# xmed-lab/NEURONS

Hardware: AMD Instinct MI355X
Metric: denoising frames/sec, 16f x 256^2 clip, 50 DDIM steps (higher is better)
Workload: dtype bf16; 1 GPU; BASELINE config 2: 1 clip(s) per call, (1,4,16,32,32) latent, 50 DDIM steps, CFG 8.5 (batch 2), SparseCtrl + temporal U-Net per step, random-init weights; clips_per_gpu=5, ddim_steps=50, hip_graph=True, output_finite=True, attention=bf16

## Files before the change

### neurons_amd/csrc/engine_ops.hip

```cpp
#include "engine.h"
#include <tuple>

using namespace nre;

struct OpScratch { void* ptr = nullptr; size_t cap = 0; };
static bool op_scratch(OpScratch& b, size_t need) {
  if (need <= b.cap) return false;
  if (b.ptr) { HIP_OK(hipDeviceSynchronize()); (void)hipFree(b.ptr); }
  b.ptr = nullptr; b.cap = 0;
  HIP_OK(hipMalloc(&b.ptr, need));
  b.cap = need;
  return true;
}

static std::map<std::tuple<const void*, int, int, int>, bf16*> g_op_fm_cache;
extern "C" void nr_op_fm_cache_clear() {
  (void)hipDeviceSynchronize();
  for (auto& kv : g_op_fm_cache) (void)hipFree(kv.second);
  g_op_fm_cache.clear();
}
static const bf16* op_pack(const NrGemmParams& p, const NrGemmRoute& r, hipStream_t s) {
  if (r.weight_layout == NR_W_ROWMAJOR || r.weight_layout == NR_W_TAP_INNER) return p.w;
  const size_t need = nr_gemm_packed_bytes(r.weight_layout, p.N, p.K);
  if (!need) throw NrError(NR_ERR_STATE, "op_pack: shape has no packed form");
  if (env_is_1("NR_OP_FM_CACHE")) {
    auto it = g_op_fm_cache.find({p.w, r.weight_layout, p.N, p.K});
    if (it == g_op_fm_cache.end()) {
      bf16* d = nullptr;
      HIP_OK(hipMalloc((void**)&d, need));
      LAUNCH_OK(nr_launch_gemm_w_pack(r.weight_layout, p.w, p.N, p.K, d, s));
      it = g_op_fm_cache.emplace(std::make_tuple(p.w, r.weight_layout, p.N, p.K), d).first;
    }
    return it->second;
  }
  static OpScratch scratch[2];
  OpScratch& b = scratch[(r.weight_layout == NR_W_FRAGMAJOR || r.weight_layout == NR_W_FRAGMAJOR_E4M3) ? 0 : 1];
  op_scratch(b, need);
  LAUNCH_OK(nr_launch_gemm_w_pack(r.weight_layout, p.w, p.N, p.K, (bf16*)b.ptr, s));
  return (const bf16*)b.ptr;
}
static void op_gemm(const NrGemmParams& p_arg, hipStream_t s) {
  NrGemmParams p = p_arg;
  p.w8 = env_is_1("NR_W8") ? 1 : 0;
  NrGemmRoute r;
  LAUNCH_OK(nr_gemm_route(&p, &r));
  const bf16* wk = op_pack(p, r, s);
  static OpScratch ws;
  op_scratch(ws, r.ws_bytes);
  LAUNCH_OK(nr_launch_gemm(&p, &r, wk, r.ws_bytes ? (float*)ws.ptr : nullptr, s));
}

extern "C" nr_status nr_op_gemm(nr_stream stream, const void* a, int32_t lda, const void* w, const float* bias,
                                const void* res, int32_t ldr, void* out, int32_t ldo, int32_t M, int32_t N, int32_t K,
                                int32_t geglu) {
  NR_TRY
  NrGemmParams p = nr_gemm_params((const bf16*)a, K, lda, nullptr, 0, 0, M, 1, 1, 1, 1, 0, (const bf16*)w, N, bias, (const bf16*)res, ldr, (bf16*)out, ldo);
  p.geglu = geglu;
  op_gemm(p, (hipStream_t)stream);
  NR_CATCH
}

extern "C" nr_status nr_op_w8_pack(nr_stream stream, const void* w_dev, int32_t N, int32_t K, void* out_dev, int64_t capacity) {
  NR_TRY
  if (!w_dev || !out_dev) throw NrError(NR_ERR_ARG, "null argument");
  const size_t need = nr_gemm_packed_bytes(NR_W_FRAGMAJOR_E4M3, N, K);
  if (!need) throw NrError(NR_ERR_ARG, "e4m3 weights: N must be a multiple of 16 and K of 64");
  if (capacity < (int64_t)need) throw NrError(NR_ERR_ARG, "output buffer too small");
  LAUNCH_OK(nr_launch_gemm_w_pack(NR_W_FRAGMAJOR_E4M3, (const bf16*)w_dev, N, K, (bf16*)out_dev, (hipStream_t)stream));
  NR_CATCH
}

extern "C" nr_status nr_op_gemm2(nr_stream stream, const void* a0, int32_t c0, int32_t lda0, const void* a1, int32_t c1, int32_t lda1,
                                 const void* w, const float* bias, const void* res, int32_t ldr, void* out, int32_t ldo, int32_t M, int32_t N) {
  NR_TRY
  NrGemmParams p = nr_gemm_params((const bf16*)a0, c0, lda0, (const bf16*)a1, c1, lda1, M, 1, 1, 1, 1, 0, (const bf16*)w, N, bias, (const bf16*)res, ldr,
                                  (bf16*)out, ldo);
  op_gemm(p, (hipStream_t)stream);
  NR_CATCH
}

extern "C" nr_status nr_op_ln_gemm(nr_stream stream, const void* a, int32_t lda, const void* w_scaled, const float* ln_c,
                                   const float* bias_folded, float eps, const void* res, int32_t ldr, void* out, int32_t ldo,
                                   int32_t M, int32_t N, int32_t K, int32_t geglu, int32_t act) {
  NR_TRY
  if (!ln_c) throw NrError(NR_ERR_ARG, "ln_c is required");
  NrGemmParams p = nr_gemm_params((const bf16*)a, K, lda, nullptr, 0, 0, M, 1, 1, 1, 1, 0, (const bf16*)w_scaled, N, bias_folded, (const bf16*)res, ldr,
                                  (bf16*)out, ldo);
  p.geglu = geglu; p.ln_c = ln_c; p.ln_eps = eps; p.act = act;
  op_gemm(p, (hipStream_t)stream);
  NR_CATCH
}

extern "C" nr_status nr_op_gemm_ex(nr_stream stream, const void* a, int32_t lda, const void* w, const float* bias, const float* ln_c,
                                   float ln_eps, const float* rowvec, int32_t rowvec_div, int32_t rowvec_mod, int32_t rowvec_ld,
                                   const void* res, int32_t ldr, void* out, int32_t ldo, int32_t M, int32_t N, int32_t K, int32_t geglu,
                                   int32_t act, float out_scale) {
  NR_TRY
  NrGemmParams p = nr_gemm_params((const bf16*)a, K, lda, nullptr, 0, 0, M, 1, 1, 1, 1, 0, (const bf16*)w, N, bias, (const bf16*)res, ldr, (bf16*)out, ldo);
  p.out_scale = out_scale; p.geglu = geglu; p.act = act;
  p.rowvec = rowvec; p.rowvec_div = rowvec_div > 0 ? rowvec_div : 1; p.rowvec_mod = rowvec_mod; p.rowvec_ld = rowvec_ld;
  p.ln_c = ln_c; p.ln_eps = ln_eps;
  op_gemm(p, (hipStream_t)stream);
  NR_CATCH
}

extern "C" nr_status nr_op_conv3x3(nr_stream stream, const void* x0, int32_t c0, const void* x1, int32_t c1, int32_t nimg,
                                   int32_t H, int32_t W, int32_t stride, int32_t ups, const void* w, const float* bias,
                                   const float* rowvec, int32_t rowvec_div, const void* res, void* out, int32_t Cout) {
  NR_TRY
  NrGemmParams p = nr_gemm_params((const bf16*)x0, c0, c0, (const bf16*)x1, c1, c1, nimg, H, W, 3, stride, ups, (const bf16*)w, Cout, bias, (const bf16*)res,
                                  Cout, (bf16*)out, Cout);
  p.rowvec = rowvec; p.rowvec_div = rowvec_div > 0 ? rowvec_div : 1; p.rowvec_ld = Cout;
  op_gemm(p, (hipStream_t)stream);
  NR_CATCH
}

extern "C" nr_status nr_op_conv3x3_ups_phase(nr_stream stream, const void* x, int32_t Cin, int32_t nimg, int32_t H, int32_t W, const void* wp,
                                             const float* bias, void* out, int32_t Cout) {
  NR_TRY
  if (!x || !wp || !out) throw NrError(NR_ERR_ARG, "null argument");
  NrGemmParams p = nr_gemm_params((const bf16*)x, Cin, Cin, nullptr, 0, 0, nimg, H, W, 3, 1, 2, (const bf16*)wp, Cout, bias, nullptr, 0, (bf16*)out, Cout);
  op_gemm(p, (hipStream_t)stream);
  NR_CATCH
}
extern "C" nr_status nr_ups_phase_weights(const float* w_tap, int32_t Cout, int32_t Cin, void* out) {
  NR_TRY
  if (!w_tap || !out || Cout < 1 || Cin < 1) throw NrError(NR_ERR_ARG, "bad argument");
  nr_ups_phase_pack(w_tap, (size_t)9 * Cin, 1, (size_t)Cin, Cout, Cin, (uint16_t*)out);
  NR_CATCH
}

extern "C" nr_status nr_op_condembed_in(nr_stream stream, const float* cond, const float* mask, int32_t c0, int32_t nsrc, int32_t F, int32_t H,
                                        int32_t W, const int32_t* fmap, int32_t nframes, const float* w, const float* bias, int32_t Cout,
                                        void* out) {
  NR_TRY
  if (!fmap) throw NrError(NR_ERR_ARG, "fmap is null");
  LAUNCH_OK(nr_launch_condembed_in(cond, mask, c0, nsrc, F, H, W, fmap, nframes, w, bias, Cout, (bf16*)out, (hipStream_t)stream));
  NR_CATCH
}

extern "C" nr_status nr_op_condembed_conv(nr_stream stream, const void* x, int32_t nimg, int32_t H, int32_t W, int32_t Cin, int32_t stride,
                                          const void* wfm, const float* bias, int32_t Cout, int32_t silu, void* out) {
  NR_TRY
  LAUNCH_OK(nr_launch_condembed_conv((const bf16*)x, nimg, H, W, Cin, stride, (const bf16*)wfm, bias, Cout, silu, (bf16*)out,
                                     (hipStream_t)stream));
  NR_CATCH
}

extern "C" nr_status nr_op_conv3x3_tap_inner(nr_stream stream, const void* x0, int32_t c0, int32_t nimg, int32_t H, int32_t W, const void* w,
                                             const float* bias, const float* rowvec, int32_t rowvec_div, const void* res, void* out,
                                             int32_t Cout) {
  NR_TRY
  NrGemmParams p = nr_gemm_params((const bf16*)x0, c0, c0, nullptr, 0, 0, nimg, H, W, 3, 1, 0, (const bf16*)w, Cout, bias, (const bf16*)res, Cout, (bf16*)out,
                                  Cout);
  p.tap_inner = 1;
  p.rowvec = rowvec; p.rowvec_div = rowvec_div > 0 ? rowvec_div : 1; p.rowvec_ld = Cout;
  op_gemm(p, (hipStream_t)stream);
  NR_CATCH
}

extern "C" nr_status nr_op_groupnorm(nr_stream stream, const void* x0, int32_t c0, const void* x1, int32_t c1, int32_t nimg,
                                     int32_t hw, int32_t groups, const float* gamma, const float* beta, float eps,
                                     int32_t silu, float* partial_ws, void* out) {
  NR_TRY
  NrGnParams p = nr_gn_params((const bf16*)x0, c0, c0, (const bf16*)x1, c1, c1, nimg, hw, groups, gamma, beta, eps, silu, partial_ws, (bf16*)out,
                              c0 + (x1 ? c1 : 0));
  NrGnRoute r;
  if (const int rc = nr_gn_route(&p, &r)) throw NrError(NR_ERR_UNSUPPORTED, "nr_gn_route -> " + std::to_string(rc) + ": no kernel serves this shape, nr_launch_groupnorm not called");
  LAUNCH_OK(nr_launch_groupnorm(&p, &r, (hipStream_t)stream));
  NR_CATCH
}

extern "C" nr_status nr_op_layernorm(nr_stream stream, const void* x, void* out, int32_t M, int32_t C, const float* gamma,
                                     const float* beta, float eps, const float* pe, int32_t pe_hw, int32_t pe_F) {
  NR_TRY
  LAUNCH_OK(nr_launch_layernorm((const bf16*)x, C, (bf16*)out, C, M, C, gamma, beta, eps, pe, pe_hw > 0 ? pe_hw : 1,
                                pe_F > 0 ? pe_F : 1, (hipStream_t)stream));
  NR_CATCH
}

extern "C" nr_status nr_op_attention(nr_stream stream, int32_t mode, const void* qp, const void* kvp, void* outp,
                                     int32_t nimg, int32_t L, int32_t Lk, int32_t C, int32_t heads, int32_t frames,
                                     int32_t kv_div) {
  NR_TRY
  const int fp8_flag = (mode & 8) ? 1 : 0;
  const int causal_flag = (mode & 16) ? 1 : 0;
  mode &= 7;
  if (causal_flag && (mode != 0 || fp8_flag)) throw NrError(NR_ERR_ARG, "causal attention: mode 0 only");
  if (mode > 2) throw NrError(NR_ERR_ARG, "bad attention mode");
  const NrAttnParams p = nr_attn_params(mode, (const bf16*)qp, (const bf16*)kvp, (bf16*)outp, mode == 1 ? C : 3 * C, 2 * C, C, nimg, L, Lk, C, heads, frames, kv_div,
                                        causal_flag, fp8_flag);
  NrAttnRoute r;
  if (const int rc = nr_attn_route(&p, &r)) throw NrError(NR_ERR_UNSUPPORTED, "nr_attn_route -> " + std::to_string(rc) + ": no kernel serves this shape, nr_launch_attention not called");
  LAUNCH_OK(nr_launch_attention(&p, &r, (hipStream_t)stream));
  NR_CATCH
}
// ... 103 lines not shown
```

### neurons_amd/csrc/gemm_route.h

```cpp
#pragma once
#include "common.h"
#include <cstdlib>
#include <initializer_list>

inline bool env_not_0(const char* name) {
  const char* v = getenv(name);
  return !(v && v[0] == '0');
}

inline int nr_plan_rows(const NrGemmParams& p) { return (p.plan_m > 0 && p.plan_m < p.M) ? p.plan_m : p.M; }

inline int nr_lds_opt_in(unsigned long long& mask, std::initializer_list<const void*> fns, size_t bytes) {
  int dev = 0;
  (void)hipGetDevice(&dev);
  const unsigned long long bit = 1ull << (dev & 63);
  if (mask & bit) return 0;
  for (const void* fn : fns)
    if (hipFuncSetAttribute(fn, hipFuncAttributeMaxDynamicSharedMemorySize, (int)bytes) != hipSuccess) return 2;
  mask |= bit;
  return 0;
}

enum NrGemmClass { NR_GEMM_SMALLM, NR_GEMM_LIN160, NR_GEMM_ROWPANEL, NR_GEMM_G8P, NR_GEMM_TILED, NR_GEMM_NCLASS };
inline const char* const nr_gemm_class_name[NR_GEMM_NCLASS] = {"smallm", "lin160", "rowpanel", "gemm8p", "tiled"};
enum NrWeightLayout { NR_W_ROWMAJOR, NR_W_TAP_INNER, NR_W_FRAGMAJOR, NR_W_LIN160, NR_W_LIN128Q, NR_W_FRAGMAJOR_E4M3 };

struct TiledPlan { int bm, bn, splitk, stages, waves, adma, lin; };
struct SmallmPlan { int nt, G, J, C; };
struct Lin160Plan { int form, big, J, cgmajor; };
struct RowPanelPlan { int nsplit; };
struct G8pPlan { int nt, phases; };

struct NrGemmRoute {
  int cls;
  int weight_layout;
  int m_fast;
  size_t ws_bytes;
  TiledPlan tiled;
  SmallmPlan smallm;
  Lin160Plan lin160;
  RowPanelPlan rowpanel;
  G8pPlan g8p;
};
```

### neurons_amd/csrc/lin160.hip

```cpp
#include "launchers.h"
#include "device_prims.h"
#include <cstdlib>

namespace {

NR_STAMP_BUF(lin160_stamp_buf, 512, 128);
#define L1_STAMP(slot) NR_STAMP_PUT(lin160_stamp_buf, slot)
#ifdef NR_STAMP_FINE
#define Q_STAMPW(slot) NR_STAMP_PUT_AT((threadIdx.x & 63) == 0 && (wave == 0 || wave == 4) && blockIdx.x < 256, lin160_stamp_buf, blockIdx.x + (wave ? 256 : 0), slot)
#else
#define Q_STAMPW(slot) do { } while (0)
#endif

constexpr int L1_BN = 160, L1_NT = 10;
constexpr int L1_W_STAGE = 24 * 1024;
constexpr int L1_NS = 3;

struct NrLin160Params {
  const bf16* x; int lda;
  const bf16* stream;
  const float* bias;
  const bf16* res; int ldr;
  bf16* out; int ldo;
  int M, N, K;
  const float* ln_c; float ln_eps;
  int norot;
};

template <int BM, int MODE = 0>
__global__ __launch_bounds__(512) void lin160_kernel(NrLin160Params p) {
  constexpr bool GLN = MODE == 1;
  static_assert(!GLN || BM == 128, "the GEGLU variant pairs the (value, gate) tiles inside one wave");
  constexpr int RT = BM / 16;
  constexpr int NTW = BM == 128 ? L1_NT : L1_NT / 2;
  constexpr int A_STAGE = BM * 128;
  constexpr int A_PW = BM == 128 ? 2 : 1;
  constexpr int STAGE = L1_W_STAGE + A_STAGE;
  constexpr int PPW = 3 + A_PW;
  extern __shared__ __attribute__((aligned(16))) unsigned char smem[];

  const int tid = threadIdx.x;
  const int lane = tid & 63;
  const int wave = __builtin_amdgcn_readfirstlane(tid >> 6);
  const int fr = lane & 15, fg = lane >> 4;
  const int rt = BM == 128 ? wave : (wave & 3);
  const int n0 = BM == 128 ? 0 : (wave >> 2) * NTW;

  L1_STAMP(0);
  const int NCB = p.N / L1_BN, S = p.K >> 6;
  const int nrg = p.M / BM;
  int rg, cb;
  if ((nrg & 7) == 0) { const int j = blockIdx.x >> 3; cb = j % NCB; rg = (j / NCB) * 8 + (int)(blockIdx.x & 7); }
  else { cb = (int)(blockIdx.x % NCB); rg = blockIdx.x / NCB; }
  const int r0 = rg * BM;
  const int rot = p.norot ? 0 : rg % S;

  const unsigned lds0 = nr_lds_addr(smem);
  const char* wsrc = reinterpret_cast<const char*>(p.stream) + (size_t)cb * ((size_t)S * L1_W_STAGE) + (size_t)(wave * 3) * 1024 + (size_t)lane * 16;
  const bf16* arow;
  {
    const int r = lane >> 2;
    arow = p.x + (size_t)(r0 + 16 * rt + r) * p.lda + (((lane & 3) ^ ((-(r >> 2)) & 3)) << 3);
  }
  auto issue_piece = [&](int s, int slot, int i) {
    const unsigned dst = lds0 + (unsigned)(slot * STAGE);
    int st = s + rot; if (st >= S) st -= S;
    if (i < 3) nr_glds16(wsrc + (size_t)st * L1_W_STAGE + (size_t)i * 1024, dst + (unsigned)((wave * 3 + i) * 1024));
    else {
      const int kk = BM == 128 ? i - 3 : (wave >> 2);
      nr_glds16(arow + 64 * st + 32 * kk, dst + (unsigned)(L1_W_STAGE + (kk * RT + rt) * 1024));
    }
  };
#pragma unroll
  for (int s = 0; s < L1_NS - 1; ++s)
#pragma unroll
    for (int i = 0; i < PPW; ++i) issue_piece(s, s, i);

  L1_STAMP(1);
  f32x4 acc[NTW];
#pragma unroll
  for (int n = 0; n < NTW; ++n) acc[n] = f32x4{0.f, 0.f, 0.f, 0.f};
  float s1 = 0.f, s2 = 0.f;
  const bf16x2 one2 = {(bf16)1.0f, (bf16)1.0f};
  const unsigned wl = (unsigned)(n0 * 1024 + lane * 16);
  const unsigned al = (unsigned)(L1_W_STAGE + rt * 1024 + fr * 64 + ((fg ^ ((-(fr >> 2)) & 3)) << 4));

  int slot = 0;
  for (int s = 0; s < S; ++s) {
    if (s + 1 < S) nr_wait_vmcnt<(L1_NS - 2) * PPW>(); else nr_wait_vmcnt<0>();
    if (s < 40) L1_STAMP(2 + 3 * s);
    __builtin_amdgcn_s_barrier();
    if (s < 40) L1_STAMP(3 + 3 * s);
    const int s_next = s + L1_NS - 1;
    const bool pf = s_next < S;
    int pslot = slot + L1_NS - 1; if (pslot >= L1_NS) pslot -= L1_NS;
    const unsigned char* base = smem + slot * STAGE;
#pragma unroll
    for (int kk = 0; kk < 2; ++kk) {
      const bf16x8 xa = *(const bf16x8*)(base + al + kk * (RT * 1024));
      if constexpr (GLN) {
#pragma unroll
        for (int e = 0; e < 4; ++e) {
          const bf16x2 pr = {xa[2 * e], xa[2 * e + 1]};
          s1 = __builtin_amdgcn_fdot2_f32_bf16(pr, one2, s1, false);
          s2 = __builtin_amdgcn_fdot2_f32_bf16(pr, pr, s2, false);
        }
      }
      bf16x8 w[NTW];
#pragma unroll
      for (int n = 0; n < NTW; ++n) w[n] = *(const bf16x8*)(base + (unsigned)((kk * L1_NT + n) * 1024) + wl);
      if (pf) {
        if (kk == 0) { issue_piece(s_next, pslot, 0); issue_piece(s_next, pslot, 1); }
        else { issue_piece(s_next, pslot, 2); issue_piece(s_next, pslot, 3); if (A_PW == 2) issue_piece(s_next, pslot, 4); }
      }
      __builtin_amdgcn_sched_barrier(0);
#pragma unroll
      for (int n = 0; n < NTW; ++n) acc[n] = __builtin_amdgcn_mfma_f32_16x16x32_bf16(w[n], xa, acc[n], 0, 0, 0);
      __builtin_amdgcn_sched_barrier(0);
    }
    if (s < 40) L1_STAMP(4 + 3 * s);
    slot = slot + 1 == L1_NS ? 0 : slot + 1;
  }
  L1_STAMP(125);

  if constexpr (GLN) {
    const float inv_k = 1.0f / (float)p.K;
    const float mu = nr_rows_sum(s1) * inv_k;
    const float rstd = rsqrtf(fmaxf(nr_rows_sum(s2) * inv_k - mu * mu, 0.f) + p.ln_eps);
    const int row = r0 + 16 * rt + fr;
    const int nb = cb * L1_BN + 4 * fg;
    bf16* orow = p.out + (size_t)row * p.ldo + cb * (L1_BN / 2) + 4 * fg;
#pragma unroll
    for (int i = 0; i < L1_NT / 2; ++i) {
      const int nv = nb + 32 * i, ng = nv + 16;
      const f32x4 cv = *(const f32x4*)(p.ln_c + nv), cg = *(const f32x4*)(p.ln_c + ng);
      const f32x4 bv = *(const f32x4*)(p.bias + nv), bg = *(const f32x4*)(p.bias + ng);
      bf16x4 o;
#pragma unroll
      for (int e = 0; e < 4; ++e) {
        const float v = (acc[2 * i][e] - mu * cv[e]) * rstd + bv[e];
        const float g = (acc[2 * i + 1][e] - mu * cg[e]) * rstd + bg[e];
        o[e] = (bf16)(v * gelu_erf_fast(g));
      }
      nr_store8(orow + 16 * i, o);
    }
    L1_STAMP(126);
    return;
  }
  const int row = r0 + 16 * rt + fr;
  const int cbase = cb * L1_BN + 16 * n0;
  bf16* orow = p.out + (size_t)row * p.ldo + cbase;
  const bf16* rrow = p.res ? p.res + (size_t)row * p.ldr + cbase : nullptr;
#pragma unroll
  for (int k = 0; k < NTW / 2; ++k) {
    f32x4 lo = acc[2 * k], hi = acc[2 * k + 1];
// ... 133 lines not shown
      f32x4 a1 = {0.f, 0.f, 0.f, 0.f}, a2 = {0.f, 0.f, 0.f, 0.f};
#pragma unroll
      for (int ks = 0; ks < KSL; ++ks) {
        a1 = __builtin_amdgcn_mfma_f32_16x16x32_bf16(ones, xb[rt][ks], a1, 0, 0, 0);
        a2 = __builtin_amdgcn_mfma_f32_16x16x32_bf16(xb[rt][ks], xb[rt][ks], a2, 0, 0, 0);
      }
      const int e_d = fr & 3;
      float d = e_d == 0 ? a2[0] : e_d == 1 ? a2[1] : e_d == 2 ? a2[2] : a2[3];
      d = (fg == (fr >> 2)) ? d : 0.f;
      sx[rt] = a1[0];
      sq2[rt] = nr_rows_sum(d);
    }
    if constexpr (KSPLIT) {
      float* xs = reinterpret_cast<float*>(smem + NS * Q_STAGE);
      if (fg == 0) {
#pragma unroll
        for (int rt = 0; rt < 2; ++rt) { xs[((wave * 2 + rt) * 2 + 0) * 16 + fr] = sx[rt]; xs[((wave * 2 + rt) * 2 + 1) * 16 + fr] = sq2[rt]; }
      }
      __builtin_amdgcn_s_barrier();
#pragma unroll
      for (int rt = 0; rt < 2; ++rt) { sx[rt] += xs[(((wave ^ 4) * 2 + rt) * 2 + 0) * 16 + fr]; sq2[rt] += xs[(((wave ^ 4) * 2 + rt) * 2 + 1) * 16 + fr]; }
    }
#pragma unroll
    for (int rt = 0; rt < 2; ++rt) {
      mu[rt] = sx[rt] * (1.0f / K);
      rstd[rt] = rsqrtf(fmaxf(sq2[rt] * (1.0f / K) - mu[rt] * mu[rt], 0.f) + p.ln_eps);
    }
  }
  L1_STAMP(127);
  nr_wait_vmcnt<0>();
  __builtin_amdgcn_s_barrier();
  L1_STAMP(1);

  const unsigned wl = (unsigned)((KSPLIT ? 16 * ch : 4 * ch) * 1024 + lane * 16);
  const unsigned oofs = (unsigned)row0 * (unsigned)p.ldo + (unsigned)((KSPLIT ? (GEGLU ? 16 * ch : 32 * ch) : (GEGLU ? 32 * ch : 64 * ch)) + 4 * fg);
  bf16x8 w[4];
#pragma unroll
  for (int n = 0; n < 4; ++n) w[n] = *(const bf16x8*)(smem + (unsigned)(n * 1024) + wl);
  f32x4 acc[2][4];
  auto epilogue = [&](int jb) {
    const int cb = cg * J + jb;
    constexpr int NF = KSPLIT ? 2 : 4;
    const float* tc = tab + jb * BN + 16 * (NF * ch) + 4 * fg;
    const float* tb = tc + J * BN;
    if constexpr (KSPLIT) {
      f32x4* ex = reinterpret_cast<f32x4*>(smem + NS * Q_STAGE);
#pragma unroll
      for (int rt = 0; rt < 2; ++rt)
#pragma unroll
        for (int nn = 0; nn < 2; ++nn) {
          f32x4 theirs;
#pragma unroll
          for (int e = 0; e < 4; ++e) theirs[e] = ch ? acc[rt][nn][e] : acc[rt][2 + nn][e];
          ex[((wave * 2 + rt) * 2 + nn) * 64 + lane] = theirs;
        }
      __builtin_amdgcn_s_barrier();
      const f32x4 c0 = *(const f32x4*)(tc), c1 = *(const f32x4*)(tc + 16), b0 = *(const f32x4*)(tb), b1 = *(const f32x4*)(tb + 16);
#pragma unroll
      for (int rt = 0; rt < 2; ++rt) {
        const f32x4 o0 = ex[(((wave ^ 4) * 2 + rt) * 2 + 0) * 64 + lane], o1 = ex[(((wave ^ 4) * 2 + rt) * 2 + 1) * 64 + lane];
        bf16x4 r0, r1;
#pragma unroll
        for (int e = 0; e < 4; ++e) {
          const float t0 = ((ch ? acc[rt][2][e] : acc[rt][0][e]) + o0[e] - mu[rt] * c0[e]) * rstd[rt] + b0[e];
          const float t1 = ((ch ? acc[rt][3][e] : acc[rt][1][e]) + o1[e] - mu[rt] * c1[e]) * rstd[rt] + b1[e];
          if constexpr (GEGLU) r0[e] = (bf16)(t0 * gelu_erf_fast(t1));
          else { r0[e] = (bf16)t0; r1[e] = (bf16)t1; }
        }
        bf16* orow = p.out + (oofs + (unsigned)(16 * rt) * (unsigned)p.ldo + (unsigned)(cb * (GEGLU ? BN / 2 : BN)));
        nr_store8(orow, r0);
        if constexpr (!GEGLU) nr_store8(orow + 16, r1);
      }
    } else if constexpr (GEGLU) {
#pragma unroll
      for (int i = 0; i < NF / 2; ++i) {
        const f32x4 cv = *(const f32x4*)(tc + 32 * i), cgv = *(const f32x4*)(tc + 32 * i + 16);
        const f32x4 bv = *(const f32x4*)(tb + 32 * i), bg = *(const f32x4*)(tb + 32 * i + 16);
#pragma unroll
        for (int rt = 0; rt < 2; ++rt) {
          bf16x4 o;
#pragma unroll
          for (int e = 0; e < 4; ++e) {
            const float v = (acc[rt][2 * i][e] - mu[rt] * cv[e]) * rstd[rt] + bv[e];
            const float gt = (acc[rt][2 * i + 1][e] - mu[rt] * cgv[e]) * rstd[rt] + bg[e];
            o[e] = (bf16)(v * gelu_erf_fast(gt));
          }
          nr_store8(p.out + (oofs + (unsigned)(16 * rt) * (unsigned)p.ldo + (unsigned)(cb * (BN / 2) + 16 * i)), o);
        }
      }
    } else {
#pragma unroll
      for (int n = 0; n < NF; ++n) {
        const f32x4 c4 = *(const f32x4*)(tc + 16 * n), b4 = *(const f32x4*)(tb + 16 * n);
#pragma unroll
        for (int rt = 0; rt < 2; ++rt) {
          bf16x4 o;
#pragma unroll
          for (int e = 0; e < 4; ++e) o[e] = (bf16)((acc[rt][n][e] - mu[rt] * c4[e]) * rstd[rt] + b4[e]);
          nr_store8(p.out + (oofs + (unsigned)(16 * rt) * (unsigned)p.ldo + (unsigned)(cb * BN + 16 * n)), o);
        }
      }
    }
  };
  const f32x4 zero4 = {0.f, 0.f, 0.f, 0.f};
  int g = 0, slot = 0;
  for (int j = 0; j < J; ++j) {
#pragma unroll
    for (int st = 0; st < S; ++st) {
      const int nslot = slot + 1 == NS ? 0 : slot + 1;
#pragma unroll
      for (int kk = 0; kk < 4; ++kk) {
        const unsigned char* nbase;
        if (kk < 3) nbase = smem + slot * Q_STAGE + (kk + 1) * (NTB * 1024);
        else {
          nr_wait_vmcnt<(NS - 2) * 4>();
          asm volatile("s_waitcnt lgkmcnt(0)" ::: "memory");
          if (g < 40) L1_STAMP(2 + 3 * g);
          __builtin_amdgcn_s_barrier();
          if (g < 40) L1_STAMP(3 + 3 * g);
          nbase = smem + nslot * Q_STAGE;
        }
        __builtin_amdgcn_sched_barrier(0);
        if (kk == 0) {
#pragma unroll
          for (int i = 0; i < 4; ++i) issue_piece(g + NS - 1, i);
        }
        __builtin_amdgcn_sched_barrier(0);
#pragma unroll
        for (int n = 0; n < 4; ++n) {
#pragma unroll
          for (int rt = 0; rt < 2; ++rt)
            acc[rt][n] = __builtin_amdgcn_mfma_f32_16x16x32_bf16(w[n], xb[rt][4 * st + kk], (st == 0 && kk == 0) ? zero4 : acc[rt][n], 0, 0, 0);
          __builtin_amdgcn_sched_barrier(0);
          w[n] = *(const bf16x8*)(nbase + (unsigned)(n * 1024) + wl);
          __builtin_amdgcn_sched_barrier(0);
        }
      }
      if (g < 40) L1_STAMP(4 + 3 * g);
      ++g;
      slot = nslot;
    }
    epilogue(j);
    if constexpr (KSPLIT) {
      __builtin_amdgcn_sched_barrier(0);
#pragma unroll
      for (int n = 0; n < 4; ++n) w[n] = *(const bf16x8*)(smem + slot * Q_STAGE + (unsigned)(n * 1024) + wl);
    }
  }
  L1_STAMP(125);
  nr_wait_vmcnt<0>();
  L1_STAMP(126);
}

__global__ __launch_bounds__(256) void lin128q_w_pack_kernel(const bf16* __restrict__ w, bf16* __restrict__ stream, int N, int K, int BN, int KPS) {
  const int S = K / (32 * KPS), CH_STAGE = Q_STAGE / 16, NTB = BN / 16;
  const long long idx = (long long)blockIdx.x * 256 + threadIdx.x;
  if (idx >= (long long)(N / BN) * S * CH_STAGE) return;
  const int cb = (int)(idx / ((long long)S * CH_STAGE));
  int c = (int)(idx - (long long)cb * S * CH_STAGE);
  const int st = c / CH_STAGE;
  c -= st * CH_STAGE;
  const int kk = c / (NTB * 64), n = (c / 64) % NTB, lane = c & 63;
  *(bf16x8*)(stream + (size_t)idx * 8) = *(const bf16x8*)(w + (size_t)(cb * BN + 16 * n + (lane & 15)) * K + 32 * (KPS * st + kk) + 8 * (lane >> 4));
}

}

#ifdef NR_STAMP
extern "C" int nr_lin160_stamp_read(void* dst, size_t bytes, int clear) { return nr_stamp_read_buf(lin160_stamp_buf, dst, bytes, clear); }
#endif

extern "C" size_t nr_lin160_stream_bytes(int N, int K) { return (N % L1_BN == 0 && K % 64 == 0) ? (size_t)(N / L1_BN) * (K / 64) * L1_W_STAGE : 0; }

extern "C" int nr_lin160_panel_rule(int Mp, int N, int K) {
  static const bool off = !env_not_0("NR_LIN160") || !env_not_0("NR_LIN160_PANEL");
  static const bool off1280 = !env_not_0("NR_LIN160_PANEL_K1280");
  static const int maxm = getenv("NR_LIN160_PANEL_MAXM") ? atoi(getenv("NR_LIN160_PANEL_MAXM")) : (1 << 30);
  if (off || Mp < 2048 || Mp > maxm || N < 3 * K) return 0;
  if (K == 640) return Mp >= 4096 && N % Q_BN == 0;
  if (K == 1280) return !off1280 && N % 64 == 0;
  return 0;
}
extern "C" size_t nr_lin128q_stream_bytes(int N, int K) {
  if (K == 640) return N % Q_BN == 0 ? (size_t)N * K * sizeof(bf16) : 0;
  if (K == 1280) return N % 64 == 0 ? (size_t)N * K * sizeof(bf16) : 0;
  return 0;
}
extern "C" int nr_launch_lin128q_w_pack(const bf16* w, int N, int K, bf16* stream, hipStream_t s) {
  const long long total = (long long)(nr_lin128q_stream_bytes(N, K) / 16);
  if (!total) return 1;
  hipLaunchKernelGGL(lin128q_w_pack_kernel, dim3((unsigned)((total + 255) / 256)), dim3(256), 0, s, w, stream, N, K, K == 1280 ? 64 : Q_BN, K == 1280 ? 8 : 4);
  return 0;
}

extern "C" bool lin160_plan(const NrGemmParams& p, Lin160Plan* pl) {
  static const bool off = !env_not_0("NR_LIN160");
  const int Mp = nr_plan_rows(p);
  *pl = Lin160Plan{0, 0, 0, 0};
  const bool ln_wide = p.ln_c && p.bias && p.ksize == 1 && p.stride == 1 && !p.ups && !p.a1 && !p.c1 && !p.rowvec && !p.act && !p.out_f32 && !p.res &&
                       p.out_scale == 1.0f && p.K == p.c0 && p.M % 128 == 0 && p.lda0 % 8 == 0 && p.ldo % 4 == 0;
  if (ln_wide && nr_lin160_panel_rule(Mp, p.N, p.K) &&
      (long long)p.M * p.ldo < (1ll << 31)) {
    const bool ksplit = p.K == 1280;
    const int bn = ksplit ? 64 : Q_BN, ncq = p.N / bn, S = 5, nrg = p.M / 128, ns = ksplit ? 3 : Q_NS;
    static const int j_force = getenv("NR_LIN160_PANEL_J") ? atoi(getenv("NR_LIN160_PANEL_J")) : 0;
    int J = 0; long long best = 0;
    for (int c = 1; c <= 16 && c <= ncq; ++c) {
      if (ncq % c != 0 || c * S < ns - 1) continue;
      const long long wgs = (long long)nrg * (ncq / c), cost = ((wgs + 255) / 256) * (c * S + 6);
      if (!J || cost <= best) { J = c; best = cost; }
    }
    if (j_force > 0 && ncq % j_force == 0 && j_force <= 16) J = j_force;
    pl->form = 4; pl->J = J;
    if (J) {
      static const int cg_force = getenv("NR_LIN160_PANEL_CGMAJOR") ? atoi(getenv("NR_LIN160_PANEL_CGMAJOR")) : -1;
      const int NCG = ncq / J;
      const double wb = 2.0 * p.N * (double)p.K, xb = 2.0 * p.M * (double)p.K;
      const bool can = NCG % 8 == 0 || 8 % NCG == 0;
      const double by_rg = 8.0 * wb + xb;
      const double by_cg = (NCG % 8 == 0 ? 1.0 : 8.0 / NCG) * wb + (NCG % 8 == 0 ? 8.0 : (double)NCG) * xb;
      pl->cgmajor = (can && by_cg < by_rg) ? 1 : 0;
      if (cg_force >= 0) pl->cgmajor = cg_force && can;
    }
    return true;
  }
  static const bool gln_on = env_not_0("NR_LIN160_GEGLU");
  if (!off && gln_on && ln_wide && p.geglu && p.K == 1280 && p.N % L1_BN == 0 && p.N >= 8192 && Mp <= 1024 && (long long)(Mp / 128) * (p.N / L1_BN) >= 192) {
    pl->form = 2;
    return true;
  }
  if (off || p.ksize != 1 || p.stride != 1 || p.ups || p.a1 || p.c1 || p.geglu || p.ln_c || p.rowvec || p.act || p.out_f32 || p.tap_inner) return false;
  if (p.out_scale != 1.0f || p.K != p.c0 || (p.K != 640 && p.K != 1280) || p.N % L1_BN != 0 || p.N > 1280) return false;
  if (p.M % 64 != 0 || Mp < 2048) return false;
  if (p.lda0 % 8 != 0 || p.ldo % 8 != 0 || (p.res && p.ldr % 8 != 0)) return false;
  if (Mp > 8192) return false;
  pl->form = 1;
  pl->big = p.M % 128 == 0 && (long long)(Mp / 128) * (p.N / L1_BN) >= 256;
  return true;
}

extern "C" int nr_launch_lin160_w_pack(const bf16* w, int N, int K, bf16* stream, hipStream_t s) {
  const long long total = (long long)(nr_lin160_stream_bytes(N, K) / 16);
  if (!total) return 1;
  hipLaunchKernelGGL(lin160_w_pack_kernel, dim3((unsigned)((total + 255) / 256)), dim3(256), 0, s, w, stream, N, K);
  return 0;
}

extern "C" int nr_launch_lin160(const NrGemmParams* pp, const Lin160Plan* pl, const bf16* stream, hipStream_t s) {
  const NrGemmParams& g = *pp;
  if (!stream) return 1;
  if (pl->form == 4) {
    const bool ksplit = g.K == 1280;
    if (!g.ln_c || !g.bias || (g.K != 640 && !ksplit) || g.M % 128 != 0 || (long long)g.M * g.ldo >= (1ll << 31)) return 1;
    const int bn = ksplit ? 64 : Q_BN, ncq = g.N / bn, nrg = g.M / 128, ns = ksplit ? 3 : Q_NS, J = pl->J;
    if (g.N % bn != 0 || J < 1 || J > 16 || ncq % J != 0) return 1;
    NrLin128QParams q;
    q.x = g.a0; q.lda = g.lda0; q.stream = stream; q.ln_c = g.ln_c; q.bias = g.bias; q.ln_eps = g.ln_eps; q.out = g.out; q.ldo = g.ldo; q.M = g.M; q.N = g.N; q.norot = g.plan_m > 0 ? 1 : 0;
    q.J = J; q.NCG = ncq / J; q.cgmajor = pl->cgmajor;
    const size_t shm_max = (size_t)Q_NS * Q_STAGE + 2 * 16 * Q_BN * sizeof(float);
    const size_t shm = (size_t)ns * Q_STAGE + (ksplit ? 32 * 1024 : 0) + (size_t)2 * J * bn * sizeof(float);
    typedef void (*kern_t)(NrLin128QParams);
    static const kern_t ks[4] = {lin128q_kernel<20, true>, lin128q_kernel<20, false>, lin128q_kernel<40, true, true>, lin128q_kernel<40, false, true>};
    static unsigned long long done[4] = {};
    const int ki = (ksplit ? 2 : 0) + (g.geglu ? 0 : 1);
    if (const int rc = nr_lds_opt_in(done[ki], {(const void*)ks[ki]}, shm_max)) return rc;
    hipLaunchKernelGGL(ks[ki], dim3((unsigned)(nrg * q.NCG)), dim3(512), shm, s, q);
    return 0;
  }
  if (g.M % 64 != 0 || g.N % L1_BN != 0 || g.K % 64 != 0 || g.K / 64 < L1_NS) return 1;
  NrLin160Params p;
  p.x = g.a0; p.lda = g.lda0; p.stream = stream; p.bias = g.bias; p.res = g.res; p.ldr = g.ldr; p.out = g.out; p.ldo = g.ldo; p.M = g.M; p.N = g.N; p.K = g.K; p.norot = g.plan_m > 0 ? 1 : 0;
  const int ncb = g.N / L1_BN;
  p.ln_c = g.ln_c; p.ln_eps = g.ln_eps;
  const bool gln = pl->form == 2, big = gln || pl->big;
  if (gln != (g.geglu != 0) || (gln && (!g.ln_c || !g.bias)) || (big && g.M % 128 != 0)) return 1;
  typedef void (*kern_t)(NrLin160Params);
  static const kern_t ks[3] = {lin160_kernel<128, 1>, lin160_kernel<128, 0>, lin160_kernel<64, 0>};
  const int ki = gln ? 0 : (big ? 1 : 2), rows = big ? 128 : 64;
  const size_t shm = (size_t)L1_NS * (L1_W_STAGE + rows * 128);
  static unsigned long long done[3] = {};
  if (const int rc = nr_lds_opt_in(done[ki], {(const void*)ks[ki]}, shm)) return rc;
  hipLaunchKernelGGL(ks[ki], dim3((unsigned)((g.M / rows) * ncb)), dim3(512), shm, s, p);
  return 0;
}
```

Measured before the change: 20.97 frames/s.

## Add LN-fused panel GEMM variant that overlaps row statistics with first weight block

Adds a new lin128q kernel variant for the non-GEGLU LayerNorm-fused panel GEMM. It loads the whole activation panel once and computes the row mean and variance with MFMA reductions (a ones vector and x·x) inside the first column block's main loop. Load issue and vmcnt waits are staged with compile-time counts so the statistics prologue overlaps with weight streaming instead of running serially. It is on by default for non-GEGLU shapes, and also adds env knobs for a minimum M and deterministic batch planning. The cost is more register pressure, extra LDS for the K-split statistics exchange, and fragile hand-tuned waitcnt arithmetic.

```diff
diff --git a/neurons_amd/csrc/engine_ops.hip b/neurons_amd/csrc/engine_ops.hip
--- a/neurons_amd/csrc/engine_ops.hip
+++ b/neurons_amd/csrc/engine_ops.hip
@@ -42,6 +42,7 @@
 static void op_gemm(const NrGemmParams& p_arg, hipStream_t s) {
   NrGemmParams p = p_arg;
   p.w8 = env_is_1("NR_W8") ? 1 : 0;
+  if (env_is_1("NR_DETERMINISTIC_BATCH")) p.plan_m = p.M;
   NrGemmRoute r;
   LAUNCH_OK(nr_gemm_route(&p, &r));
   const bf16* wk = op_pack(p, r, s);
diff --git a/neurons_amd/csrc/gemm_route.h b/neurons_amd/csrc/gemm_route.h
--- a/neurons_amd/csrc/gemm_route.h
+++ b/neurons_amd/csrc/gemm_route.h
@@ -27,7 +27,7 @@
 
 struct TiledPlan { int bm, bn, splitk, stages, waves, adma, lin; };
 struct SmallmPlan { int nt, G, J, C; };
-struct Lin160Plan { int form, big, J, cgmajor; };
+struct Lin160Plan { int form; union { int big; int early; }; int J, cgmajor; };
 struct RowPanelPlan { int nsplit; };
 struct G8pPlan { int nt, phases; };
 
diff --git a/neurons_amd/csrc/lin160.hip b/neurons_amd/csrc/lin160.hip
--- a/neurons_amd/csrc/lin160.hip
+++ b/neurons_amd/csrc/lin160.hip
@@ -1,6 +1,7 @@
 #include "launchers.h"
 #include "device_prims.h"
 #include <cstdlib>
+#include <type_traits>
 
 namespace {
 
@@ -440,6 +441,272 @@
   L1_STAMP(126);
 }
 
+
+template <int... I, class F> __device__ __forceinline__ void q_static_for(std::integer_sequence<int, I...>, F&& f) { (f(std::integral_constant<int, I>{}), ...); }
+constexpr int q_grp(int s, int S) { return s < S ? 12 : 4; }
+constexpr int q_younger(int from, int to, int S) { int n = 0; for (int s = from; s <= to; ++s) n += q_grp(s, S); return n; }
+constexpr int q_hi(int st, int S, int NS) { return st < S - 1 ? st + 2 : S + NS - 2; }
+constexpr int q_wait_x(int st, int kk, int S, int NS) { return 6 - 2 * kk + q_younger(st + 1, q_hi(st, S, NS), S); }
+constexpr int q_wait_w(int st, int S, int NS) { return (st + 1 < S ? 8 : 0) + q_younger(st + 2, q_hi(st, S, NS), S); }
+
+template <int KS, bool GEGLU, bool KSPLIT = false>
+__global__ __launch_bounds__(512) void lin128q_early_kernel(NrLin128QParams p) {
+  constexpr int K = 32 * KS;
+  constexpr int KSL = KSPLIT ? KS / 2 : KS;
+  constexpr int KPS = KSPLIT ? 8 : 4;
+  constexpr int S = KS / KPS;
+  constexpr int BN = KSPLIT ? 64 : Q_BN, NTB = BN / 16;
+  constexpr int NS = KSPLIT ? 3 : Q_NS;
+  constexpr int XCH = KSPLIT ? 32 * 1024 : 0;
+  static_assert(KSL == 20 && S == 5, "20 k-steps per wave in 5 stages of 4");
+  extern __shared__ __attribute__((aligned(16))) unsigned char smem[];
+  const int tid = threadIdx.x;
+  const int lane = tid & 63;
+  const int wave = __builtin_amdgcn_readfirstlane(tid >> 6);
+  const int fr = lane & 15, fg = lane >> 4;
+  const int rp = wave & 3, ch = wave >> 2;
+  L1_STAMP(0);
+  const int J = p.J;
+  int rg, cg;
+  const int nrg = p.M >> 7;
+  if (!p.cgmajor && (nrg & 7) == 0) { const int i = blockIdx.x >> 3; cg = i % p.NCG; rg = (i / p.NCG) * 8 + (int)(blockIdx.x & 7); }
+  else { cg = (int)(blockIdx.x % p.NCG); rg = (int)(blockIdx.x / p.NCG); }
+  const int row0 = rg * 128 + 32 * rp + fr;
+  const int rot = p.norot ? 0 : rg % S;
+  const int G = J * S;
+
+  const unsigned lds0 = nr_lds_addr(smem);
+  const char* wbase = reinterpret_cast<const char*>(p.stream) + (size_t)cg * J * ((size_t)S * Q_STAGE) + (size_t)(wave * 4) * 1024 + (size_t)lane * 16;
+  auto issue_piece = [&](int g, int i) {
+    const int gs = g < G ? g : G - 1;
+    const int j = gs / S;
+    int st = gs - j * S + rot; if (st >= S) st -= S;
+    nr_glds16(wbase + ((size_t)j * S + st) * Q_STAGE + (size_t)i * 1024, lds0 + (unsigned)((g % NS) * Q_STAGE + (wave * 4 + i) * 1024));
+  };
+  float* tab = reinterpret_cast<float*>(smem + NS * Q_STAGE + XCH);
+  bf16x8 xb[2][KSL];
+  const bf16* xr[2];
+#pragma unroll
+  for (int rt = 0; rt < 2; ++rt) xr[rt] = p.x + (size_t)(row0 + 16 * rt) * p.lda + 8 * fg + (KSPLIT ? 128 * ch : 0);
+  auto issue_panel = [&](int st) {
+    int sq = st + rot; if (sq >= S) sq -= S;
+#pragma unroll
+    for (int kk = 0; kk < 4; ++kk)
+#pragma unroll
+      for (int rt = 0; rt < 2; ++rt)
+        asm volatile("global_load_dwordx4 %0, %1, off" : "=v"(xb[rt][4 * st + kk]) : "v"(xr[rt] + 32 * (KPS * sq + kk)) : "memory");
+  };
+  float mu[2], rstd[2], sx[2], sq2[2];
+  f32x4 sa1[2] = {{0.f, 0.f, 0.f, 0.f}, {0.f, 0.f, 0.f, 0.f}}, sa2[2] = {{0.f, 0.f, 0.f, 0.f}, {0.f, 0.f, 0.f, 0.f}};
+  bf16x8 ones;
+#pragma unroll
+  for (int e = 0; e < 8; ++e) ones[e] = (bf16)1.0f;
+  auto stats_step = [&](int rt, int ks) {
+    sa1[rt] = __builtin_amdgcn_mfma_f32_16x16x32_bf16(ones, xb[rt][ks], sa1[rt], 0, 0, 0);
+    sa2[rt] = __builtin_amdgcn_mfma_f32_16x16x32_bf16(xb[rt][ks], xb[rt][ks], sa2[rt], 0, 0, 0);
+  };
+  auto stats_rows = [&]() {
+#pragma unroll
+    for (int rt = 0; rt < 2; ++rt) {
+      const int e_d = fr & 3;
+      float d = e_d == 0 ? sa2[rt][0] : e_d == 1 ? sa2[rt][1] : e_d == 2 ? sa2[rt][2] : sa2[rt][3];
+      d = (fg == (fr >> 2)) ? d : 0.f;
+      sx[rt] = sa1[rt][0];
+      sq2[rt] = nr_rows_sum(d);
+    }
+  };
+  float* xs = reinterpret_cast<float*>(smem + NS * Q_STAGE + XCH + 2 * J * BN * sizeof(float));
+  auto stats_put = [&]() {
+    if (fg == 0) {
+#pragma unroll
+      for (int rt = 0; rt < 2; ++rt) { xs[((wave * 2 + rt) * 2 + 0) * 16 + fr] = sx[rt]; xs[((wave * 2 + rt) * 2 + 1) * 16 + fr] = sq2[rt]; }
+    }
+  };
+  auto stats_get = [&]() {
+#pragma unroll
+    for (int rt = 0; rt < 2; ++rt) { sx[rt] += xs[(((wave ^ 4) * 2 + rt) * 2 + 0) * 16 + fr]; sq2[rt] += xs[(((wave ^ 4) * 2 + rt) * 2 + 1) * 16 + fr]; }
+  };
+  auto stats_final = [&]() {
+#pragma unroll
+    for (int rt = 0; rt < 2; ++rt) {
+      mu[rt] = sx[rt] * (1.0f / K);
+      rstd[rt] = rsqrtf(fmaxf(sq2[rt] * (1.0f / K) - mu[rt] * mu[rt], 0.f) + p.ln_eps);
+    }
+  };
+
+  {
+    const int n4 = (J * BN) >> 2, tq = tid < n4 ? tid : n4 - 1;
+    f32x4 tc, tb;
+    asm volatile("global_load_dwordx4 %0, %1, off" : "=v"(tc) : "v"(p.ln_c + cg * J * BN + 4 * tq) : "memory");
+    asm volatile("global_load_dwordx4 %0, %1, off" : "=v"(tb) : "v"(p.bias + cg * J * BN + 4 * tq) : "memory");
+#pragma unroll
+    for (int g = 0; g <= q_hi(-1, S, NS); ++g) {
+#pragma unroll
+      for (int i = 0; i < 4; ++i) issue_piece(g, i);
+      issue_panel(g);
+    }
+    L1_STAMP(122);
+    asm volatile("s_waitcnt vmcnt(%2)" : "+v"(tc), "+v"(tb) : "n"(q_wait_w(-1, S, NS)) : "memory");
+    if (tid < n4) { *(f32x4*)(tab + 4 * tid) = tc; *(f32x4*)(tab + J * BN + 4 * tid) = tb; }
+    L1_STAMP(123);
+    __builtin_amdgcn_s_barrier();
+  }
+  L1_STAMP(1);
+
+  const unsigned wl = (unsigned)((KSPLIT ? 16 * ch : 4 * ch) * 1024 + lane * 16);
+  const unsigned oofs = (unsigned)row0 * (unsigned)p.ldo + (unsigned)((KSPLIT ? (GEGLU ? 16 * ch : 32 * ch) : (GEGLU ? 32 * ch : 64 * ch)) + 4 * fg);
+  bf16x8 w[4];
+#pragma unroll
+  for (int n = 0; n < 4; ++n) w[n] = *(const bf16x8*)(smem + (unsigned)(n * 1024) + wl);
+  f32x4 acc[2][4];
+  auto epilogue = [&](int jb, auto with_stats) {
+    constexpr bool STATS = decltype(with_stats)::value;
+    if constexpr (STATS) stats_rows();
+    if constexpr (STATS && !KSPLIT) { stats_final(); L1_STAMP(127); }
+    const int cb = cg * J + jb;
+    constexpr int NF = KSPLIT ? 2 : 4;
+    const float* tc = tab + jb * BN + 16 * (NF * ch) + 4 * fg;
+    const float* tb = tc + J * BN;
+    if constexpr (KSPLIT) {
+      f32x4* ex = reinterpret_cast<f32x4*>(smem + NS * Q_STAGE);
+#pragma unroll
+      for (int rt = 0; rt < 2; ++rt)
+#pragma unroll
+        for (int nn = 0; nn < 2; ++nn) {
+          f32x4 theirs;
+#pragma unroll
+          for (int e = 0; e < 4; ++e) theirs[e] = ch ? acc[rt][nn][e] : acc[rt][2 + nn][e];
+          ex[((wave * 2 + rt) * 2 + nn) * 64 + lane] = theirs;
+        }
+      if constexpr (STATS) stats_put();
+      __builtin_amdgcn_s_barrier();
+      if constexpr (STATS) { stats_get(); stats_final(); L1_STAMP(127); }
+      const f32x4 c0 = *(const f32x4*)(tc), c1 = *(const f32x4*)(tc + 16), b0 = *(const f32x4*)(tb), b1 = *(const f32x4*)(tb + 16);
+#pragma unroll
+      for (int rt = 0; rt < 2; ++rt) {
+        const f32x4 o0 = ex[(((wave ^ 4) * 2 + rt) * 2 + 0) * 64 + lane], o1 = ex[(((wave ^ 4) * 2 + rt) * 2 + 1) * 64 + lane];
+        bf16x4 r0, r1;
+#pragma unroll
+        for (int e = 0; e < 4; ++e) {
+          const float t0 = ((ch ? acc[rt][2][e] : acc[rt][0][e]) + o0[e] - mu[rt] * c0[e]) * rstd[rt] + b0[e];
+          const float t1 = ((ch ? acc[rt][3][e] : acc[rt][1][e]) + o1[e] - mu[rt] * c1[e]) * rstd[rt] + b1[e];
+          if constexpr (GEGLU) r0[e] = (bf16)(t0 * gelu_erf_fast(t1));
+          else { r0[e] = (bf16)t0; r1[e] = (bf16)t1; }
+        }
+        bf16* orow = p.out + (oofs + (unsigned)(16 * rt) * (unsigned)p.ldo + (unsigned)(cb * (GEGLU ? BN / 2 : BN)));
+        nr_store8(orow, r0);
+        if constexpr (!GEGLU) nr_store8(orow + 16, r1);
+      }
+    } else if constexpr (GEGLU) {
+#pragma unroll
+      for (int i = 0; i < NF / 2; ++i) {
+        const f32x4 cv = *(const f32x4*)(tc + 32 * i), cgv = *(const f32x4*)(tc + 32 * i + 16);
+        const f32x4 bv = *(const f32x4*)(tb + 32 * i), bg = *(const f32x4*)(tb + 32 * i + 16);
+#pragma unroll
+        for (int rt = 0; rt < 2; ++rt) {
+          bf16x4 o;
+#pragma unroll
+          for (int e = 0; e < 4; ++e) {
+            const float v = (acc[rt][2 * i][e] - mu[rt] * cv[e]) * rstd[rt] + bv[e];
+            const float gt = (acc[rt][2 * i + 1][e] - mu[rt] * cgv[e]) * rstd[rt] + bg[e];
+            o[e] = (bf16)(v * gelu_erf_fast(gt));
+          }
+          nr_store8(p.out + (oofs + (unsigned)(16 * rt) * (unsigned)p.ldo + (unsigned)(cb * (BN / 2) + 16 * i)), o);
+        }
+      }
+    } else {
+#pragma unroll
+      for (int n = 0; n < NF; ++n) {
+        const f32x4 c4 = *(const f32x4*)(tc + 16 * n), b4 = *(const f32x4*)(tb + 16 * n);
+#pragma unroll
+        for (int rt = 0; rt < 2; ++rt) {
+          bf16x4 o;
+#pragma unroll
+          for (int e = 0; e < 4; ++e) o[e] = (bf16)((acc[rt][n][e] - mu[rt] * c4[e]) * rstd[rt] + b4[e]);
+          nr_store8(p.out + (oofs + (unsigned)(16 * rt) * (unsigned)p.ldo + (unsigned)(cb * BN + 16 * n)), o);
+        }
+      }
+    }
+  };
+  const f32x4 zero4 = {0.f, 0.f, 0.f, 0.f};
+  int g = 0, slot = 0;
+  auto block = [&](auto first) {
+    constexpr bool FIRST = decltype(first)::value;
+    q_static_for(std::make_integer_sequence<int, S>{}, [&](auto st_c) {
+      constexpr int st = decltype(st_c)::value;
+      const int nslot = slot + 1 == NS ? 0 : slot + 1;
+      q_static_for(std::make_integer_sequence<int, 4>{}, [&](auto kk_c) {
+        constexpr int kk = decltype(kk_c)::value;
+        const unsigned char* nbase;
+        if (kk < 3) nbase = smem + slot * Q_STAGE + (kk + 1) * (NTB * 1024);
+        else {
+          nr_wait_vmcnt<FIRST ? q_wait_w(st, S, NS) : (NS - 2) * 4>();
+          asm volatile("s_waitcnt lgkmcnt(0)" ::: "memory");
+          if (g < 40) L1_STAMP(2 + 3 * g);
+          __builtin_amdgcn_s_barrier();
+          if (g < 40) L1_STAMP(3 + 3 * g);
+          if constexpr (FIRST) { if (st == S - 1) L1_STAMP(124); }
+          nbase = smem + nslot * Q_STAGE;
+        }
+        __builtin_amdgcn_sched_barrier(0);
+        if constexpr (FIRST) {
+          if (kk == 0) {
+#pragma unroll
+            for (int gi = q_hi(st - 1, S, NS) + 1; gi <= q_hi(st, S, NS); ++gi) {
+#pragma unroll
+              for (int i = 0; i < 4; ++i) issue_piece(gi, i);
+              if (gi < S) issue_panel(gi);
+            }
+          }
+        } else if (kk == 0) {
+#pragma unroll
+          for (int i = 0; i < 4; ++i) issue_piece(g + NS - 1, i);
+        }
+        __builtin_amdgcn_sched_barrier(0);
+        if constexpr (FIRST) {
+          asm volatile("s_waitcnt vmcnt(%2)" : "+v"(xb[0][4 * st + kk]), "+v"(xb[1][4 * st + kk]) : "n"(q_wait_x(st, kk, S, NS)) : "memory");
+          __builtin_amdgcn_sched_barrier(0);
+        }
+#pragma unroll
+        for (int n = 0; n < 4; ++n) {
+#pragma unroll
+          for (int rt = 0; rt < 2; ++rt)
+            acc[rt][n] = __builtin_amdgcn_mfma_f32_16x16x32_bf16(w[n], xb[rt][4 * st + kk], (st == 0 && kk == 0) ? zero4 : acc[rt][n], 0, 0, 0);
+          __builtin_amdgcn_sched_barrier(0);
+          w[n] = *(const bf16x8*)(nbase + (unsigned)(n * 1024) + wl);
+          __builtin_amdgcn_sched_barrier(0);
+        }
+        if constexpr (FIRST) {
+#pragma unroll
+          for (int rt = 0; rt < 2; ++rt) stats_step(rt, 4 * st + kk);
+          __builtin_amdgcn_sched_barrier(0);
+        }
+      });
+      if (g < 40) L1_STAMP(4 + 3 * g);
+      ++g;
+      slot = nslot;
+    });
+  };
+  auto refill = [&]() {
+    if constexpr (KSPLIT) {
+      __builtin_amdgcn_sched_barrier(0);
+#pragma unroll
+      for (int n = 0; n < 4; ++n) w[n] = *(const bf16x8*)(smem + slot * Q_STAGE + (unsigned)(n * 1024) + wl);
+    }
+  };
+  block(std::true_type{});
+  epilogue(0, std::true_type{});
+  refill();
+  for (int j = 1; j < J; ++j) {
+    block(std::false_type{});
+    epilogue(j, std::false_type{});
+    refill();
+  }
+  L1_STAMP(125);
+  nr_wait_vmcnt<0>();
+  L1_STAMP(126);
+}
+
 __global__ __launch_bounds__(256) void lin128q_w_pack_kernel(const bf16* __restrict__ w, bf16* __restrict__ stream, int N, int K, int BN, int KPS) {
   const int S = K / (32 * KPS), CH_STAGE = Q_STAGE / 16, NTB = BN / 16;
   const long long idx = (long long)blockIdx.x * 256 + threadIdx.x;
@@ -464,8 +731,9 @@
   static const bool off = !env_not_0("NR_LIN160") || !env_not_0("NR_LIN160_PANEL");
   static const bool off1280 = !env_not_0("NR_LIN160_PANEL_K1280");
   static const int maxm = getenv("NR_LIN160_PANEL_MAXM") ? atoi(getenv("NR_LIN160_PANEL_MAXM")) : (1 << 30);
-  if (off || Mp < 2048 || Mp > maxm || N < 3 * K) return 0;
-  if (K == 640) return Mp >= 4096 && N % Q_BN == 0;
+  static const int minm = getenv("NR_LIN160_PANEL_MINM") ? atoi(getenv("NR_LIN160_PANEL_MINM")) : 0;
+  if (off || Mp < (minm > 0 ? minm : 2048) || Mp > maxm || N < 3 * K) return 0;
+  if (K == 640) return Mp >= (minm > 0 ? minm : 4096) && N % Q_BN == 0;
   if (K == 1280) return !off1280 && N % 64 == 0;
   return 0;
 }
@@ -484,7 +752,7 @@
 extern "C" bool lin160_plan(const NrGemmParams& p, Lin160Plan* pl) {
   static const bool off = !env_not_0("NR_LIN160");
   const int Mp = nr_plan_rows(p);
-  *pl = Lin160Plan{0, 0, 0, 0};
+  *pl = Lin160Plan{};
   const bool ln_wide = p.ln_c && p.bias && p.ksize == 1 && p.stride == 1 && !p.ups && !p.a1 && !p.c1 && !p.rowvec && !p.act && !p.out_f32 && !p.res &&
                        p.out_scale == 1.0f && p.K == p.c0 && p.M % 128 == 0 && p.lda0 % 8 == 0 && p.ldo % 4 == 0;
   if (ln_wide && nr_lin160_panel_rule(Mp, p.N, p.K) &&
@@ -499,7 +767,10 @@
       if (!J || cost <= best) { J = c; best = cost; }
     }
     if (j_force > 0 && ncq % j_force == 0 && j_force <= 16) J = j_force;
+    static const bool early_on = env_not_0("NR_LIN128Q_PROLOGUE");
+    const bool early = early_on && !p.geglu;
     pl->form = 4; pl->J = J;
+    pl->early = early ? 1 : 0;
     if (J) {
       static const int cg_force = getenv("NR_LIN160_PANEL_CGMAJOR") ? atoi(getenv("NR_LIN160_PANEL_CGMAJOR")) : -1;
       const int NCG = ncq / J;
@@ -546,11 +817,14 @@
     q.x = g.a0; q.lda = g.lda0; q.stream = stream; q.ln_c = g.ln_c; q.bias = g.bias; q.ln_eps = g.ln_eps; q.out = g.out; q.ldo = g.ldo; q.M = g.M; q.N = g.N; q.norot = g.plan_m > 0 ? 1 : 0;
     q.J = J; q.NCG = ncq / J; q.cgmajor = pl->cgmajor;
     const size_t shm_max = (size_t)Q_NS * Q_STAGE + 2 * 16 * Q_BN * sizeof(float);
-    const size_t shm = (size_t)ns * Q_STAGE + (ksplit ? 32 * 1024 : 0) + (size_t)2 * J * bn * sizeof(float);
+    const bool early = pl->early != 0;
+    const size_t shm = (size_t)ns * Q_STAGE + (ksplit ? 32 * 1024 : 0) + (size_t)2 * J * bn * sizeof(float) + (ksplit && early ? 2048 : 0);
     typedef void (*kern_t)(NrLin128QParams);
-    static const kern_t ks[4] = {lin128q_kernel<20, true>, lin128q_kernel<20, false>, lin128q_kernel<40, true, true>, lin128q_kernel<40, false, true>};
-    static unsigned long long done[4] = {};
-    const int ki = (ksplit ? 2 : 0) + (g.geglu ? 0 : 1);
+    static const kern_t ks[6] = {lin128q_kernel<20, true>, lin128q_kernel<20, false>, lin128q_kernel<40, true, true>, lin128q_kernel<40, false, true>,
+                                 lin128q_early_kernel<20, false>, lin128q_early_kernel<40, false, true>};
+    static unsigned long long done[6] = {};
+    if (early && g.geglu) return 1;
+    const int ki = early ? (ksplit ? 5 : 4) : (ksplit ? 2 : 0) + (g.geglu ? 0 : 1);
     if (const int rc = nr_lds_opt_in(done[ki], {(const void*)ks[ki]}, shm_max)) return rc;
     hipLaunchKernelGGL(ks[ki], dim3((unsigned)(nrg * q.NCG)), dim3(512), shm, s, q);
     return 0;
```

Result: no change. 20.96 frames/s (-0.0%).
